# leggedrobotics/raisimLib

Measured on AMD Instinct MI355X. Metric: env-steps/sec, 4096 ANYmal-C envs flat terrain dt=0.0025, higher is better.
Workload: dtype f32

## Files before the change

### raisimlib_amd/csrc/rsb_world.hip

```cpp
#include <dlfcn.h>
#include <hip/hip_runtime.h>

#include <algorithm>
#include <cmath>
#include <cstdio>
#include <cstdlib>
#include <chrono>
#include <cstring>
#include <memory>
#include <string>
#include <vector>

#include "query_kernel.h"
#include "rsb.h"
#include "rsb_internal.h"
#include "step_launch.h"
#include "env_task.h"
#include "step_types.h"


#include "rsb_world.h"
#include "rsb_spec.h"

namespace rsbw {

struct DevKernargDefault { DevKernargDefault() { setenv("HIP_FORCE_DEV_KERNARG", "1", 0); setenv("GPU_MAX_HW_QUEUES", "8", 0); } } g_dev_kernarg_default;

int round4(int x) { return (x + 3) & ~3; }

void build_dev_model(const rsb_model_blob& b, DevModel* d) {
  std::memset(d, 0, sizeof *d);
  d->nb = b.nb; d->nq = b.nq; d->nv = b.nv; d->ncol = b.ncol; d->depth = b.depth;
  d->cw = round4(6 + b.depth - 1);
  d->fixed_base = b.fixed_base;
  std::vector<std::vector<int>> kids(b.nb);
  for (int i = 0; i < b.nb; ++i) {
    d->parent[i] = b.parent[i]; d->level[i] = b.level[i]; d->jtype[i] = b.jtype[i];
    if (i > 0) kids[b.parent[i]].push_back(i);
    float* f = d->bodyf[i];
    for (int c = 0; c < 3; ++c) {
      d->axis[i][c] = f[c] = (float)b.axis[i][c];
      d->ptree[i][c] = f[4 + c] = (float)b.ptree[i][c];
      d->com[i][c] = f[17 + c] = (float)b.com[i][c];
    }
    std::memcpy(&f[3], &b.jtype[i], sizeof(int));
    for (int c = 0; c < 9; ++c) d->rtree[i][c] = f[8 + c] = (float)b.rtree[i][c];
    for (int c = 0; c < 6; ++c) d->inertia[i][c] = f[20 + c] = (float)b.inertia[i][c];
    d->mass[i] = f[7] = (float)b.mass[i];
    d->armature[i] = f[26] = (float)b.armature[i];
    f[27] = (float)b.damping[i];
    f[28] = (float)b.effort[i];
    const bool limited = i > 0 && b.q_lower[i] < b.q_upper[i] && b.q_lower[i] > -1e29 && b.q_upper[i] < 1e29;
    f[29] = limited ? (float)b.q_lower[i] : -3e38f;
    f[30] = limited ? (float)b.q_upper[i] : 3e38f;
  }
  for (int i = 0; i < b.nb * b.depth; ++i) d->anc[i] = -1;
  for (int i = 0; i < b.nb; ++i)
    for (int j = i; j >= 0; j = b.parent[j]) d->anc[i * b.depth + b.level[j]] = j;
  int pos = 0;
  d->max_kid = 0;
  for (int i = 0; i < b.nb; ++i) {
    d->kid_start[i] = pos;
    d->kid_count[i] = (int)kids[i].size();
    for (int c : kids[i]) d->kid_list[pos++] = c;
    if (i >= 1 && d->kid_count[i] > d->max_kid) d->max_kid = d->kid_count[i];
  }
  for (int s = 0; s < b.ncol; ++s) {
    d->col_body[s] = b.col_body[s];
    for (int c = 0; c < 3; ++c) d->col_pos[s][c] = (float)b.col_pos[s][c];
    d->col_pos[s][3] = (float)b.col_radius[s];
  }
}

std::vector<int> enumerate_self_pairs(const rsb_model_blob& b, const std::vector<uint8_t>& ignore) {
  std::vector<int> out;
  for (int i = 0; i < b.ncol; ++i)
    for (int j = i + 1; j < b.ncol; ++j) {
      const int bi = b.col_body[i], bj = b.col_body[j];
      if (bi == bj || b.parent[bi] == bj || b.parent[bj] == bi) continue;
      if (b.col_rim[i] > 0.0 || b.col_rim[j] > 0.0) continue;
      if (!(b.col_radius[i] + b.col_radius[j] > 0.0)) continue;
      if (!ignore.empty() && (ignore[bi * b.nb + bj] || ignore[bj * b.nb + bi])) continue;
      out.push_back(i); out.push_back(j);
    }
  return out;
}

int up_quad_table(const rsb_model_blob& b, int* table) {
  if (b.nb > 16 || b.depth < 2 || b.nb - 1 != 4 * (b.depth - 1)) return 0;
  int first[4], n1 = 0;
  for (int i = 1; i < b.nb; ++i) {
    if (b.level[i] == 1) { if (n1 == 4) return 0; first[n1++] = i; }
    else if (b.parent[i] != i - 1) return 0;
  }
  if (n1 != 4) return 0;
  for (int g = 0; g < 4; ++g)
    for (int lv = 1; lv < b.depth; ++lv) {
      const int body = first[g] + lv - 1;
      if (body >= b.nb || b.level[body] != lv) return 0;
      if (table) table[(lv - 1) * 4 + g] = body;
    }
  return b.depth - 1;
}

int hm_slots_for(const rsb_model_blob& b) { return std::max(rsbk::kHmSlots, (int)b.ncol); }

int kcap_of(const rsb_model_blob& b, int kmax) { return (kmax <= 8 && b.depth - 1 <= 4) ? 8 : 16; }

static LdsLayout make_layout_pitch(const rsb_model_blob& b, int kcap, int n_self, int model_pitch) {
  LdsLayout L;
  L.model_pitch = model_pitch;
  const int cw = round4(6 + b.depth - 1);
  int o = 0;
  auto take = [&](int n) { int r = o; o += round4(n); return r; };
  L.t_model = take(b.nb * model_pitch);
  L.t_gain = take(2 * b.nb);
  L.t_parlv = take(b.nb);
  L.t_anc = take(b.nb * b.depth);
  L.t_dir = take(64);
  L.t_col = take(rsbk::kColSlot * b.ncol);
  L.t_kids = take(b.nb);
  L.t_kidx = take(b.nb);
  L.t_spair = take(n_self > 0 ? n_self + 1 : 0);
  L.shared_total = o;
  o = 0;
  L.q = take(b.nq < 8 ? 8 : b.nq); L.u = take(b.nv < 8 ? 8 : b.nv);
  L.pt = take(b.nq); L.dtg = take(b.nv); L.tf = take(b.nv < 8 ? 8 : b.nv);
  L.body = take(b.nb * rsbk::kBodySlot);
  const bool tri = kcap > 8;
  if (!tri) L.fact = take(b.nb * rsbk::kFactSlot);
  L.wb = take(b.nv);
  L.con = take(kcap * rsbk::kConSlot);
  L.wc = take(3 * kcap * cw);
  L.cv = take(3 * kcap);
  L.gstride = 4 * kcap + 4;
  static_assert(rsbk::g_row_pitch(8) <= 3 * (4 * 8 + 4), "the block rows of the Delassus phase must fit the region of the dense rows");
  const int gsize = tri ? (kcap * (kcap + 1) / 2) * 12 : 3 * kcap * L.gstride;
  const int upsize = b.nb * rsbk::kUpSlot + (tri ? b.nb * rsbk::kFactSlot : 0);
  L.g = take(std::max({gsize, upsize, (rsbk::kHmRec + 8) * hm_slots_for(b) + RSB_MAX_COLLISIONS + 16}));
  if (tri) L.fact = L.g + b.nb * rsbk::kUpSlot;
  L.ginv = take(12 * kcap);
  L.lam = take(3 * kcap);
  L.warm = take(6 * b.ncol);
  L.tact = take(b.nv);
  L.cen = L.wc; L.selft = 0;
  if (n_self > 0) {
    if (4 * b.ncol > 3 * kcap * cw) L.cen = take(4 * b.ncol);
    L.selft = take(4 * kcap);
  }
  L.per_env = o + rsbk::kEnvPad;
  return L;
}

static size_t lds_bytes_of(const LdsLayout& L, int lpe) { return sizeof(float) * ((size_t)L.shared_total + (size_t)(64 / lpe) * L.per_env); }

LdsLayout make_layout(const rsb_model_blob& b, int kcap, int n_self) {
  const LdsLayout tight = make_layout_pitch(b, kcap, n_self, rsbk::kModelSlot), wide = make_layout_pitch(b, kcap, n_self, rsbk::kModelPitch);
  auto wgs = [](const LdsLayout& L, int lpe) {
    const size_t bytes = lds_bytes_of(L, lpe);
    return bytes > 160 * 1024 ? 0 : (int)std::min<size_t>(4, (160 * 1024) / bytes);
  };
  for (int lpe : {16, 32, 64}) if (wgs(wide, lpe) != wgs(tight, lpe)) return tight;
  return wide;
}

size_t lds_bytes_for(const rsb_model_blob& b, int kcap, int lpe, int n_self) { return lds_bytes_of(make_layout(b, kcap, n_self), lpe); }

int default_lpe(const rsb_model_blob& b, int kmax, int n_self) {
  const int kcap = kcap_of(b, kmax);
  const int need = b.nb > 16 ? (b.nb > 32 ? 64 : 32) : 16;
  int best = 64, best_envs = 0, best_wgs = 0;
  for (int lpe = need; lpe <= 64; lpe *= 2) {
    const size_t wg = lds_bytes_for(b, kcap, lpe, n_self);
    if (wg > 160 * 1024) continue;
    if (n_self > 30 * lpe) continue;
    const int wgs = (int)std::min<size_t>(4, (160 * 1024) / wg);
    const int envs = wgs * (64 / lpe);
    if (envs > best_envs || (envs == best_envs && wgs > best_wgs)) { best_envs = envs; best_wgs = wgs; best = lpe; }
  }
  return best;
}

__global__ void warm_clear_kernel(float* warm, const uint8_t* mask, int N, int n6) {
  const int i = blockIdx.x * blockDim.x + threadIdx.x;
  if (i >= N * n6) return;
// ... 192 lines not shown

std::vector<float> build_lds_image(const rsb_world* w, const LdsLayout& L, bool rk4_contact) {
  const rsb_model_blob& b = w->blob;
  auto dm = std::make_unique<DevModel>();
  build_dev_model(b, dm.get());
  std::vector<float> img((size_t)L.shared_total, 0.f);
  auto put_i = [&](int off, int v) { std::memcpy(&img[off], &v, sizeof(int)); };
  for (int i = 0; i < b.nb; ++i) {
    for (int c = 0; c < rsbk::kModelSlot; ++c) img[L.t_model + i * L.model_pitch + c] = dm->bodyf[i][c];
    if (rk4_contact) img[L.t_model + i * L.model_pitch + 28] = 0.f;
    const bool pd = w->control_mode == RSB_PD_PLUS_FEEDFORWARD_TORQUE && !rk4_contact && i >= 1;
    img[L.t_gain + 2 * i] = pd ? w->h_kp[i + 5] : 0.f;
    img[L.t_gain + 2 * i + 1] = pd ? w->h_kd[i + 5] : 0.f;
    put_i(L.t_parlv + i, (b.parent[i] + 1) | (b.level[i] << 8));
    put_i(L.t_kids + i, dm->kid_list[i]);
    put_i(L.t_kidx + i, dm->kid_start[i] | (dm->kid_count[i] << 16));
  }
  for (int i = 0; i < b.nb * b.depth; ++i) put_i(L.t_anc + i, dm->anc[i]);
  for (int k = 0; k < 16; ++k) {
    const double lo = ((k + 15) & 15) * 0.125 * M_PI, hi = ((k + 1) & 15) * 0.125 * M_PI;
    img[L.t_dir + 4 * k] = (float)std::cos(lo); img[L.t_dir + 4 * k + 1] = (float)std::sin(lo);
    img[L.t_dir + 4 * k + 2] = (float)std::cos(hi); img[L.t_dir + 4 * k + 3] = (float)std::sin(hi);
  }
  for (int i = 0; i < b.ncol; ++i) {
    float* ct = &img[L.t_col + rsbk::kColSlot * i];
    ct[0] = (float)b.col_pos[i][0]; ct[1] = (float)b.col_pos[i][1]; ct[2] = (float)b.col_pos[i][2]; ct[3] = (float)b.col_radius[i];
    put_i(L.t_col + rsbk::kColSlot * i + 4, b.col_body[i]);
    ct[8] = (float)b.col_axis[i][0]; ct[9] = (float)b.col_axis[i][1]; ct[10] = (float)b.col_axis[i][2]; ct[11] = (float)b.col_rim[i];
    ct[5] = (float)(w->col_mu[i] >= 0 ? w->col_mu[i] : w->mu);
    ct[6] = (float)(w->col_rest[i] >= 0 ? w->col_rest[i] : w->restitution);
    ct[7] = (float)(w->col_rthr[i] >= 0 ? w->col_rthr[i] : w->res_threshold);
  }
  for (int k = 0; k < n_self_pairs(w); ++k) put_i(L.t_spair + k, (16 * w->self_pairs[2 * k]) | ((16 * w->self_pairs[2 * k + 1]) << 16));
  return img;
}

int upload_image(rsb_world* w, const LdsLayout& L, bool rk4_contact) {
  if (!w->image_dirty && rk4_contact == w->image_rk4_contact && std::memcmp(&L, &w->image_layout, sizeof L) == 0) return RSB_OK;
    std::vector<float> img = build_lds_image(w, L, rk4_contact);
    HIP_TRY(hipMemcpyAsync(w->d_image, img.data(), img.size() * sizeof(float), hipMemcpyHostToDevice, stream_of(w)));
    const int np = n_self_pairs(w);
    std::vector<float> mat((size_t)4 * np, 0.f);
    for (int k = 0; k < np; ++k) {
      mat[4 * k] = (float)(w->self_mu[k] >= 0 ? w->self_mu[k] : w->mu);
      mat[4 * k + 1] = (float)(w->self_rest[k] >= 0 ? w->self_rest[k] : w->restitution);
      mat[4 * k + 2] = (float)(w->self_rthr[k] >= 0 ? w->self_rthr[k] : w->res_threshold);
    }
    if (np > 0) {
      if ((size_t)np > w->self_mat_cap) {
        if (w->d_self_mat) HIP_TRY(hipFree(w->d_self_mat));
        w->d_self_mat = nullptr; w->self_mat_cap = 0;
        HIP_TRY(hipMalloc(&w->d_self_mat, (size_t)4 * np * sizeof(float)));
        w->self_mat_cap = (size_t)np;
      }
      HIP_TRY(hipMemcpyAsync(w->d_self_mat, mat.data(), mat.size() * sizeof(float), hipMemcpyHostToDevice, stream_of(w)));
    }
    HIP_TRY(hipStreamSynchronize(stream_of(w)));
    w->image_dirty = false;
    w->image_layout = L; w->image_rk4_contact = rk4_contact;
  return RSB_OK;
}

void fill_world_args(const rsb_world* w, const LdsLayout& L, const StepClass& c, StepArgs& a) {
  a.model = w->d_model;
  a.gc = w->d_gc; a.gv = w->d_gv; a.ptarget = w->d_pt; a.dtarget = w->d_dt; a.tauff = w->d_tff;
#ifndef RSB_X_READ_ZERO_ROWS
  if (w->dt_zero && !w->raw_dt) a.dtarget = nullptr;
  if (w->tff_zero && !w->raw_tff) a.tauff = nullptr;
#endif
  a.kp = w->d_kp; a.kd = w->d_kd;
  a.contacts = w->d_contacts; a.contact_count = w->d_count; a.flags = w->d_flags; a.iters = w->d_iters;
  a.heights = w->d_heights;
  a.hm_index = w->d_hm_index;
  a.warm = w->warm_start ? w->d_warm : nullptr;
  a.lds_image = w->d_image; a.L = L; a.lds_floats = (int)(lds_bytes_of(L, c.lpe) / sizeof(float));
  a.gc0 = w->d_gc; a.gv0 = w->d_gv; a.reset_rows = w->N;
  a.tau_out = w->want_genf ? w->d_genf : nullptr;
  a.prof = w->d_prof;
  a.dbg = w->dbg_env >= 0 ? w->d_dbg : nullptr;
  a.dbg_env = w->dbg_env;
  a.N = w->N; a.kmax = w->kmax; a.control_mode = w->control_mode;
  a.nb = w->blob.nb; a.nq = w->blob.nq; a.nv = w->blob.nv; a.ncol = w->blob.ncol; a.depth = w->blob.depth;
  a.cw = round4(6 + w->blob.depth - 1); a.max_kid = w->max_kid; a.fixed_base = w->blob.fixed_base; a.chain = (w->chain && c.lpe == 16) ? 1 : 0;
  if (a.chain && c.kmax <= 8 && up_quad_table(w->blob, nullptr) > 0 && w->blob.nb * rsbk::kUpQuadSlot <= L.ginv - L.g) a.chain = 2;
  a.dt = (float)w->dt; a.gx = (float)w->gravity[0]; a.gy = (float)w->gravity[1]; a.gz = (float)w->gravity[2];
  a.mu = (float)w->mu; a.erp = (float)w->erp;
  a.alpha_init = (float)w->alpha_init; a.alpha_min = (float)w->alpha_min; a.alpha_decay = (float)w->alpha_decay;
  a.threshold = (float)w->threshold; a.max_iter = w->max_iter; a.section_rounds = w->section_rounds;
  a.multi_depth = w->multi_depth; a.multi_light = w->multi_light; a.multi_freeze_after = w->multi_freeze_after; a.multi_stall_window = w->multi_stall_window;
  a.anderson = w->kmax > 8 ? w->anderson : 0;
  a.anderson_clip = (float)w->anderson_clip;
  a.hm_contacts = w->hm_contacts; a.hm_second_cos = (float)w->hm_second_cos; a.hm_slots = hm_slots_for(w->blob);
  a.hm_capsule = w->hm_capsule ? w->n_cap : 0; a.hm_cap = w->d_cap;
  a.integ_theta = (float)w->integ_theta;
  a.stall_window = w->stall_window; a.stall_factor = (float)w->stall_factor; a.freeze_after = w->freeze_after; a.refine = w->refine; a.settle_tol = (float)w->settle_tol; a.restitution = (float)w->restitution; a.res_threshold = (float)w->res_threshold;
  a.terrain_type = w->terrain_type; a.hm_xs = w->hm_xs; a.hm_ys = w->hm_ys; a.ground_z = (float)w->ground_z;
  if (w->terrain_type == 1) {
    double dx = w->hm_xsize / (w->hm_xs - 1), dy = w->hm_ysize / (w->hm_ys - 1);
    a.hm_x0 = (float)(w->hm_cx - 0.5 * w->hm_xsize); a.hm_y0 = (float)(w->hm_cy - 0.5 * w->hm_ysize);
    a.hm_dx = (float)dx; a.hm_dy = (float)dy; a.hm_inv_dx = (float)(1.0 / dx); a.hm_inv_dy = (float)(1.0 / dy);
    a.hm_max = w->hm_max;
  }
  a.n_self = n_self_pairs(w); a.self_mat = w->d_self_mat;
  static const bool poison = std::getenv("RSB_POISON_LDS") != nullptr;
  a.poison_lds = poison ? 1 : 0;
  static const bool prof_fine = std::getenv("RSB_PROF_FINE") != nullptr;
  a.prof_fine = prof_fine ? 1 : 0;
}

void apply_request(rsb_world* w, const StepRequest& f, StepArgs& a) {
  if (f.rk4_contact) { a.control_mode = RSB_FORCE_AND_TORQUE; a.integ_theta = 1.f; a.tauff = w->d_tff; }
  if (f.ptarget_src) { a.ptarget = f.ptarget_src; a.ptarget_store = w->d_pt; }
  if (f.act) { a.act = f.act; a.act_mean = w->d_env_mean; a.act_std = w->env_cfg.action_std; a.ptarget_store = w->d_pt; a.tau2_out = w->d_env_tau2; }
  if (f.env_task) {
    a.env_reward = f.env_reward; a.env_ob = f.env_ob;
    a.env_fwd_coeff = w->env_cfg.forward_vel_coeff; a.env_fwd_clip = w->env_cfg.forward_vel_clip;
    a.env_torque_coeff = w->env_cfg.torque_coeff; a.env_terminal_reward = w->env_cfg.terminal_reward;
    a.tau2_out = nullptr;
  }
  a.obs_out = f.obs_out; a.obs_idx = f.obs_idx; a.obs_slots = f.obs_slots;
  if (f.peer) {
    rsb_world::Peer& P = w->peer;
    const uint32_t step = ++P.step;
    const int par = (int)(step & 1u);
    const size_t bufsz = (size_t)P.ranks * w->N * P.od;
    for (int p = 0; p < P.ranks; ++p) {
      float* pb = static_cast<float*>(P.peer_base[p]);
      a.obs_peer[p] = pb + (size_t)par * bufsz;
      a.obs_flag[p] = reinterpret_cast<uint32_t*>(pb + 2 * bufsz) + (size_t)par * RSB_MAX_RANKS + P.rank;
    }
    a.obs_ctr = reinterpret_cast<uint32_t*>(static_cast<float*>(P.base) + 2 * bufsz) + 2 * RSB_MAX_RANKS;
    a.n_obs_peers = P.ranks; a.obs_row0 = P.rank * w->N; a.obs_step = step;
    a.obs_slots = P.slots; a.obs_idx = P.idx.empty() ? nullptr : P.d_idx;
  }
  a.early_term = (w->early_term && f.have_allowed) ? 1 : 0; a.allowed = f.allowed;
  if (f.do_reset) { a.do_reset = f.do_reset; a.gc0 = f.gc0; a.gv0 = f.gv0; a.reset_rows = f.rows; }
  if (f.res_steps > 0) {
    a.res_steps = f.res_steps; a.res_full = w->res_full ? 1 : 0;
    a.res_targets = f.res_targets; a.res_period = f.res_period; a.res_first = f.res_first;
    a.res_obs_stride = f.res_obs_stride; a.res_done_stride = f.res_done_stride; a.res_pass_global0 = f.res_pass_global0;
    if (f.res_stage == 1) a.res_pol.lin = f.res_lin;
    if (f.res_stage == 2) a.res_pol.mlp = f.res_mlp;
    if (f.res_stage == 0) { a.ptarget = f.res_targets + (size_t)(f.res_first % f.res_period) * ((size_t)w->N * w->blob.nq); a.ptarget_store = w->d_pt; }
  }
  a.done_out = f.redirect_done ? f.done_out : w->d_done_out;
  a.env_mask = f.mask;
}

int enqueue_step(rsb_world* w, const StepRequest& f, bool pipelined, const StepClass& c, StepArgs& a) {
  const int blocks = (w->N + 64 / c.lpe - 1) / (64 / c.lpe);
  hipStream_t ls = nullptr;
  if (pipelined) {
    int st = pipe_begin_launch(w, a, blocks, f.closed_loop, &ls);
    if (st != RSB_OK) return st;
    if (!f.closed_loop) {
      rsb_world::PipeLog e;
      e.req = f; e.nsub = a.nsub; e.req.pipeline = false;
      if (!f.redirect_done) { e.req.redirect_done = true; e.req.done_out = w->d_done_out; }
      w->pipe_log.push_back(e);
    }
    w->pipe_time_logged += a.nsub * w->dt;
  } else {
    ls = stream_of(w);
    if (w->pipe_dep) { HIP_TRY(hipStreamWaitEvent(ls, w->pipe_dep, 0)); w->pipe_dep = nullptr; }
  }
  hipEvent_t e0 = w->ev0, e1 = w->ev1;
  const bool rec = w->timing && (w->launch_index++ % w->timing_stride == 0);
// ... 1169 lines not shown
```

### raisimlib_amd/csrc/step_kernel.h

```cpp
#pragma once

#include <hip/hip_runtime.h>
#include <stdint.h>

#include <type_traits>

#include "env_task.h"
#include "rsb_types.h"
#include "step_types.h"
#include "step_spec.h"
#include "step_math.h"
#include "step_terrain.h"
#include "step_slip.h"
#include "step_slip_pk.h"
#include "stage_bodies.h"

#ifndef RSB_X_RES_RING
#define RSB_X_RES_RING 0
#endif
#if defined(RSB_I_CL) && ((RSB_I_CL) & 64)
#define RSB_RESIDENT 1
#else
#define RSB_RESIDENT 0
#endif
// ... 145 lines not shown
    if (a.pipe_xcds > 0) {
      unsigned xcc;
      asm volatile("s_getreg_b32 %0, hwreg(HW_REG_XCC_ID)" : "=s"(xcc));
      xcc &= 15u;
      unsigned t = 0;
      if (lane == 0) t = __hip_atomic_fetch_add(a.pipe_xcc_ctr + (xcc << 6), 1u, __ATOMIC_RELAXED, __HIP_MEMORY_SCOPE_AGENT) - a.pipe_xcc_base;
      t = (unsigned)__builtin_amdgcn_readfirstlane((int)t);
      const unsigned per = gridDim.x / (unsigned)a.pipe_xcds;
      if (t >= per || xcc >= (unsigned)a.pipe_xcds) {
        if (lane == 0 && atomicCAS(a.pipe_err, 0, 1 ) == 0) __hip_atomic_store(a.pipe_err_host, 1, __ATOMIC_RELAXED, __HIP_MEMORY_SCOPE_SYSTEM);
        return;
      }
      blk = (int)(xcc * per + t);
    }
  }
  int env = blk * EPW + el;
  bool env_valid = env < a.N;
  if (!env_valid) env = a.N - 1;
  if (a.env_mask && !a.env_mask[env]) env_valid = false;
  const int nb = RSB_DIM(NB, a.nb), nq = RSB_DIM(NQ, a.nq), nv = RSB_DIM(NV, a.nv), depth = RSB_DIM(DEPTH, a.depth), ncol = RSB_DIM(NCOL, a.ncol);
#ifdef RSB_SPECIALIZED
  constexpr int cw = (6 + RSB_SPEC_DEPTH - 1 + 3) & ~3;
#else
  const int cw = a.cw;
#endif
  const bool fixed_base = RSB_DIM(FIXED_BASE, a.fixed_base != 0);
  const auto& L = a.L;

  float* MODELF = lds + L.t_model;
  float* GAIN = lds + L.t_gain;
  int* PARLV = reinterpret_cast<int*>(lds + L.t_parlv);
  int* ANC = reinterpret_cast<int*>(lds + L.t_anc);
  float* DIR16 = lds + L.t_dir;
  float* COLT = lds + L.t_col;
  int* KIDS = reinterpret_cast<int*>(lds + L.t_kids);
  int* KIDX = reinterpret_cast<int*>(lds + L.t_kidx);
  float* E = lds + L.shared_total + el * L.per_env;
  float* Q = E + L.q;
  float* U = E + L.u;
  float* PT = E + L.pt;
  float* DTG = E + L.dtg;
  float* TF = E + L.tf;
  float* BODY = E + L.body;
  float* UPS = E + L.g;
  float* FACT = E + L.fact;
  float* WB = E + L.wb;
  float* CON = E + L.con;
  float* WC = E + L.wc;
  float* CV = E + L.cv;
  float* G = E + L.g;
  float* GINV = E + L.ginv;
  float* LAM = E + L.lam;
  float* TACT = E + L.tact;
  float* WARM = E + L.warm;
  const int* SPAIR = reinterpret_cast<const int*>(lds + L.t_spair);
  float* CEN = E + L.cen;
  float* SELFT = E + L.selft;
  const int n_self = RSB_DIM(N_SELF, a.n_self);
  const int nwarm = 6 * ncol;
  const int GS = L.gstride;

  if (PROF && a.poison_lds) {
    for (int i = lane; i < a.lds_floats; i += 64) lds[i] = __int_as_float(0x7fc00000);
    __syncthreads();
  }
#if RSB_RESIDENT
#if RSB_SPEC_CONSTS
  int ncs_pin = a.res_steps;
  asm volatile("" : "+s"(ncs_pin));
  const int ncs = ncs_pin;
#else
  const int ncs = a.res_steps;
#endif
  if constexpr (STG != 0) resident_stage<STG, EPW>(ka, blk, 0, ncs);
#endif
#include "step_phase_prologue.inc"
#if RSB_SEAM_CARRY
  [[maybe_unused]] float sc_q = 0.f, sc_qd = 0.f;
  [[maybe_unused]] float sc_qv[7], sc_uv[6];
#endif
#if RSB_LEAN_SEAM
#include "step_phase_seam_setup.inc"
#endif
#if RSB_RESIDENT
  for (int cs = 0; cs < ncs; ++cs) {
#endif
#if RSB_SEAM_CARRY
#if RSB_LEAN_SEAM
  if (seam_refill)
#endif
  {
#if RSB_SEAM_BASE
    float t0[8], t1[8];
    ldv<2>(Q, t0); ldv<2>(U, t1);
#endif
#if RSB_SEAM_JOINTS
    const float jq = Q[bb + 6], jqd = U[bb + 5];
    sc_q = isbody ? jq : 0.f; sc_qd = isbody ? jqd : 0.f;
#endif
#if RSB_SEAM_BASE
    RSB_UNROLL for (int i = 0; i < 7; ++i) sc_qv[i] = t0[i];
    RSB_UNROLL for (int i = 0; i < 6; ++i) sc_uv[i] = t1[i];
#endif
  }
#endif
  for (int sub = 0; sub < nsub; ++sub) {
    RSB_STAMP(0)
    RSB_ARGS(ab);
    tsq = 0.f;
#include "step_phase_tree_down.inc"
#include "step_phase_collision.inc"
#include "step_phase_tree_up.inc"
    iters_used = 0;
    float wlam[6] = {0.f, 0.f, 0.f, 0.f, 0.f, 0.f};
    if (ncw > 0) {
      RSB_ARGS(aw);
      const float erp = RSB_DIM_F32(ERP, aw.erp);
#include "step_phase_columns.inc"
#include "step_phase_delassus.inc"
#include "step_phase_solver.inc"
    } else if (has_warm) {
      for (int i = s; i < nwarm; i += LPE) WARM[i] = 0.f;
    }
    RSB_STAMP(6)

#include "step_phase_update.inc"
  }

  if (PROF && a.prof && lane == 0) { long long* P = a.prof + 16 + 16 * (long long)blk; P[8] = t_setup; P[9] = t_newt; P[10] = t_epi; P[11] = t_rule; P[12] = t_exch; P[13] = t_end; P[14] = t_start - t_entry; P[15] = t_mag; P[0] = clock64() - t_start; P[1] = t_gs; P[2] = p_iters; P[3] = p_ncw; P[4] = p_search; P[5] = p_newton; P[6] = p_solves; P[7] = t_srch; }
#if RSB_LEAN_SEAM
  if (ls_ok && cs + 1 < ncs) {
#include "step_phase_seam_lean.inc"
  } else {
    seam_refill = true;
    asm volatile("; rsb generic seam begin");
#endif
#include "step_phase_epilogue.inc"
#if RSB_LEAN_SEAM
    asm volatile("; rsb generic seam end");
  }
#endif
#if RSB_RESIDENT
  }
#endif
}

}
```

### raisimlib_amd/csrc/step_phase_delassus.inc

```
      const int npw = ncw * (ncw + 1) / 2;
      for (int p0 = 0; p0 < npw; p0 += LPE) {
        const int p = p0 + s;
        const int j = (int)((__builtin_sqrtf(8.0f * (float)p + 1.5f) - 1.0f) * 0.5f);
        const int i = p - ((j * (j + 1)) >> 1);
        if (j < nc) {
          const int bi = __float_as_int(CON[i * kConSlot + 7]), bj = __float_as_int(CON[j * kConSlot + 7]);
          const int li = PARLV[bi] >> 8, lj = PARLV[bj] >> 8;
          int ai[ML], aj[ML];
#if defined(RSB_SPECIALIZED) && RSB_SPEC_DEPTH == 4
          {
            const int4 ri = *reinterpret_cast<const int4*>(ANC + bi * 4), rj = *reinterpret_cast<const int4*>(ANC + bj * 4);
            const int vi[4] = {ri.y, ri.z, ri.w, -1}, vj[4] = {rj.y, rj.z, rj.w, -2};
            RSB_UNROLL for (int l = 0; l < ML; ++l) {
              ai[l] = (l + 1 <= li && l < 3) ? vi[l < 3 ? l : 3] : -1;
              aj[l] = (l + 1 <= lj && l < 3) ? vj[l < 3 ? l : 3] : -2;
            }
          }
#else
          RSB_UNROLL for (int l = 0; l < ML; ++l) {
            ai[l] = (l + 1 <= li) ? ANC[bi * depth + l + 1] : -1;
            aj[l] = (l + 1 <= lj) ? ANC[bj * depth + l + 1] : -2;
          }
#endif
          int lca = 0;
          bool same = true;
          RSB_UNROLL for (int l = 0; l < ML; ++l) { same = same && (ai[l] == aj[l]); lca += same ? 1 : 0; }
#if RSB_FLAT_SETUP_HEAD
          constexpr int CWC = 6 + RSB_SPEC_DEPTH - 1;
#else
          constexpr int CWC = 6 + ML;
#endif
          float wi[3][CWC], wj[3][CWC];
          const float* Wi = WC + (3 * i) * cw;
          const float* Wj = WC + (3 * j) * cw;
          RSB_UNROLL for (int rr = 0; rr < 3; ++rr) {
            RSB_UNROLL for (int q4 = 0; q4 < (CWC + 3) / 4; ++q4) {
              float t4[4], u4[4];
              ld4(Wi + rr * cw + 4 * q4, t4); ld4(Wj + rr * cw + 4 * q4, u4);
              RSB_UNROLL for (int e = 0; e < 4; ++e)
                if (4 * q4 + e < CWC) { wi[rr][4 * q4 + e] = t4[e]; wj[rr][4 * q4 + e] = u4[e]; }
            }
          }
          float acc[9];
          RSB_UNROLL for (int q2 = 0; q2 < 9; ++q2) acc[q2] = 0.f;
          RSB_UNROLL for (int e = 0; e < CWC; ++e) {
            const bool on = e < 6 || e < 6 + lca;
            float av[3], bv[3];
            RSB_UNROLL for (int rr = 0; rr < 3; ++rr) { av[rr] = on ? wi[rr][e] : 0.f; bv[rr] = on ? wj[rr][e] : 0.f; }
            RSB_UNROLL for (int rr = 0; rr < 3; ++rr)
              RSB_UNROLL for (int cc = 0; cc < 3; ++cc) acc[3 * rr + cc] += av[rr] * bv[cc];
          }
          if (i == j && CON[i * kConSlot + 15] != 0.f) { acc[0] = 1.f; acc[4] = 1.f; }
          if constexpr (TRI) {
            float* bp = G + tri_off(j, i);
            RSB_UNROLL for (int cc = 0; cc < 3; ++cc) {
              const float row[4] = {acc[cc], acc[3 + cc], acc[6 + cc], 0.f};
              st4(bp + 4 * cc, row);
            }
          } else if constexpr (GROWS) {
            const float B[3][3] = {{acc[0], acc[1], acc[2]}, {acc[3], acc[4], acc[5]}, {acc[6], acc[7], acc[8]}};
            const float Bt[3][3] = {{acc[0], acc[3], acc[6]}, {acc[1], acc[4], acc[7]}, {acc[2], acc[5], acc[8]}};
            gblk_store(G + i * GRP + kGBlock * j, B);
            if (i != j) gblk_store(G + j * GRP + kGBlock * i, Bt);
          } else {
            RSB_UNROLL for (int rr = 0; rr < 3; ++rr)
              RSB_UNROLL for (int cc = 0; cc < 3; ++cc) {
                G[(3 * i + rr) * GS + 4 * j + cc] = acc[3 * rr + cc];
                G[(3 * j + cc) * GS + 4 * i + rr] = acc[3 * rr + cc];
              }
          }
          if (i == j) {
            float gi[12];
            inv3(acc, gi);
            gi[9] = gi[10] = gi[11] = 0.f;
            stv<3>(GINV + 12 * i, gi);
          }
        }
      }
      __syncthreads();
      if constexpr (FIXED) {
        if (s < nc && __float_as_int(CON[s * kConSlot + 11]) < kSelfA) {
          float acc[9], gi[12];
          float* dg = TRI ? G + tri_off(s, s) : (GROWS ? G + s * GRP + kGBlock * s : G + 3 * s * GS + 4 * s);
          const int dgs = TRI ? 4 : GS;
          if constexpr (GROWS) {
            float D[3][3];
            gblk_load(dg, D);
            RSB_UNROLL for (int rr = 0; rr < 3; ++rr) RSB_UNROLL for (int cc = 0; cc < 3; ++cc) acc[3 * rr + cc] = D[rr][cc];
          } else {
            RSB_UNROLL for (int rr = 0; rr < 3; ++rr) {
              float g4[4];
              ld4(dg + rr * dgs, g4);
              acc[3 * rr] = g4[0]; acc[3 * rr + 1] = g4[1]; acc[3 * rr + 2] = g4[2];
            }
          }
          const float reg = kSelfReg * (acc[0] + acc[4] + acc[8]) * (1.0f / 3.0f);
          RSB_UNROLL for (int rr = 0; rr < 3; ++rr) { acc[4 * rr] += reg; dg[GROWS ? g_block_off(rr, rr) : rr * dgs + rr] = acc[4 * rr]; }
          inv3(acc, gi);
          gi[9] = gi[10] = gi[11] = 0.f;
          stv<3>(GINV + 12 * s, gi);
        }
        __syncthreads();
      }
      if (__any(nselfc > 0)) {
        for (int sa = 0; sa + 1 < ncw; ++sa) {
          const bool prim = sa + 1 < nc && (__float_as_int(CON[sa * kConSlot + 11]) & kSelfA) != 0;
          if (!__any(prim)) continue;
          const int sb = sa + 1;
          const float z4[4] = {0.f, 0.f, 0.f, 0.f};
          if constexpr (TRI) {
            if (prim && s < nc) {
              float A[3][3], B[3][3];
              const float Z[3][3] = {{0.f, 0.f, 0.f}, {0.f, 0.f, 0.f}, {0.f, 0.f, 0.f}};
              if (s != sa && s != sb) {
                tri_load(G, sa, s, A); tri_load(G, sb, s, B);
                RSB_UNROLL for (int r = 0; r < 3; ++r) RSB_UNROLL for (int c = 0; c < 3; ++c) A[r][c] += B[r][c];
                tri_store(G, sa, s, A); tri_store(G, sb, s, Z);
              } else if (s == sa) {
                float X[3][3], D[3][3];
                tri_load(G, sa, sa, A); tri_load(G, sb, sb, B); tri_load(G, sb, sa, X);
                RSB_UNROLL for (int r = 0; r < 3; ++r) RSB_UNROLL for (int c = 0; c < 3; ++c) D[r][c] = A[r][c] + B[r][c] + X[r][c] + X[c][r];
                const float ju = SELFT[4 * sa + 3] + SELFT[4 * sb + 3];
                float m4[4];
                ld4(SELFT + 4 * sa, m4);
                RSB_UNROLL for (int rr = 0; rr < 3; ++rr) { CV[3 * sa + rr] += CV[3 * sb + rr]; CV[3 * sb + rr] = 0.f; }
                if (m4[1] > 0.f && ju < -m4[2]) CV[3 * sa + 2] += m4[1] * ju;
                const float reg = (FIXED ? 2.f : 1.f) * kSelfReg * (D[0][0] + D[1][1] + D[2][2]) * (1.0f / 3.0f);
                RSB_UNROLL for (int rr = 0; rr < 3; ++rr) D[rr][rr] += reg;
                const float I3[3][3] = {{1.f, 0.f, 0.f}, {0.f, 1.f, 0.f}, {0.f, 0.f, 1.f}};
                tri_store(G, sa, sa, D); tri_store(G, sb, sa, Z); tri_store(G, sb, sb, I3);
                float acc[9], gi[12];
                RSB_UNROLL for (int r = 0; r < 3; ++r) RSB_UNROLL for (int c = 0; c < 3; ++c) acc[3 * r + c] = D[r][c];
                inv3(acc, gi);
                gi[9] = gi[10] = gi[11] = 0.f;
                stv<3>(GINV + 12 * sa, gi);
                RSB_UNROLL for (int q2 = 0; q2 < 12; ++q2) gi[q2] = 0.f;
                gi[0] = gi[4] = gi[8] = 1.f;
                stv<3>(GINV + 12 * sb, gi);
              }
            }
            __syncthreads();
            continue;
          }
          if (prim && s < nc) {
            if constexpr (GROWS) {
              gblk_add(G + sa * GRP + kGBlock * s, G + sb * GRP + kGBlock * s);
            } else {
              RSB_UNROLL for (int rr = 0; rr < 3; ++rr) {
                float ga[4], gb[4];
                ld4(G + (3 * sa + rr) * GS + 4 * s, ga); ld4(G + (3 * sb + rr) * GS + 4 * s, gb);
                RSB_UNROLL for (int e = 0; e < 4; ++e) ga[e] += gb[e];
                st4(G + (3 * sa + rr) * GS + 4 * s, ga); st4(G + (3 * sb + rr) * GS + 4 * s, z4);
              }
            }
          }
          __syncthreads();
          if constexpr (GROWS) {
            if (prim && s < nc) gblk_add(G + s * GRP + kGBlock * sa, G + s * GRP + kGBlock * sb);
          } else if (prim) {
            for (int r = s; r < 3 * nc; r += LPE) {
              float ga[4], gb[4];
// ... 38 lines not shown
```

### raisimlib_amd/csrc/step_spec.h

```cpp
#pragma once

#define RSB_SPEC_FIELDS(X)                                                                                                              \
  X(NB, a.nb) X(NQ, a.nq) X(NV, a.nv) X(DEPTH, a.depth) X(NCOL, a.ncol) X(MAX_KID, a.max_kid) X(FIXED_BASE, (a.fixed_base != 0))      \
  X(N_SELF, a.n_self) X(NSUB, a.nsub) X(KMAX, a.kmax) X(HAS_WARM, (a.warm != nullptr)) X(TERRAIN, a.terrain_type)                      \
  X(EARLY_TERM, (a.early_term != 0)) X(SECTION_ROUNDS, a.section_rounds) X(STALL_WINDOW, a.stall_window) X(FREEZE_AFTER, a.freeze_after) \
  X(REFINE, a.refine) X(MULTI_FA, a.multi_freeze_after) X(MULTI_DEPTH, a.multi_depth) X(MULTI_LIGHT, a.multi_light)                    \
  X(MULTI_SW, a.multi_stall_window) X(CHAIN, (a.chain != 0)) X(MODEL_PITCH, a.L.model_pitch) \
  X(UP_QUADS, (a.chain == 2)) \
  X(MU, rsbk::spec_bits(a.mu)) X(ERP, rsbk::spec_bits(a.erp)) X(ALPHA_INIT, rsbk::spec_bits(a.alpha_init)) X(ALPHA_MIN, rsbk::spec_bits(a.alpha_min)) \
  X(ALPHA_DECAY, rsbk::spec_bits(a.alpha_decay)) X(THRESHOLD, rsbk::spec_bits(a.threshold)) X(STALL_FACTOR, rsbk::spec_bits(a.stall_factor)) \
  X(MAX_ITER, a.max_iter)

#ifdef RSB_SPECIALIZED
#define RSB_DIM(NAME, expr) (RSB_SPEC_##NAME)
#else
#define RSB_DIM(NAME, expr) (expr)
#endif

namespace rsbk {
constexpr int spec_bits(float f) { return __builtin_bit_cast(int, f); }
constexpr float spec_f32(int bits) { return __builtin_bit_cast(float, bits); }
}
#if defined(RSB_SPECIALIZED) && !defined(RSB_X_NO_SPEC_CONSTS)
#define RSB_SPEC_CONSTS 1
// ... 12 lines not shown
#endif
#else
#define RSB_UP_QUADS 0
#endif

#if RSB_UP_QUADS && !defined(RSB_X_NO_DOWN_QUADS)
#define RSB_DOWN_QUADS 1
#else
#define RSB_DOWN_QUADS 0
#endif

#if RSB_DOWN_QUADS && !defined(RSB_X_NO_SEAM_CARRY)
#define RSB_SEAM_CARRY 1
#else
#define RSB_SEAM_CARRY 0
#endif
#if RSB_SEAM_CARRY && !defined(RSB_X_NO_SEAM_JOINTS)
#define RSB_SEAM_JOINTS 1
#else
#define RSB_SEAM_JOINTS 0
#endif
#if RSB_SEAM_CARRY && !defined(RSB_X_NO_SEAM_BASE)
#define RSB_SEAM_BASE 1
#else
#define RSB_SEAM_BASE 0
#endif
#if RSB_SEAM_CARRY && !defined(RSB_X_NO_SEAM_LOADS)
#define RSB_SEAM_LOADS 1
#else
#define RSB_SEAM_LOADS 0
#endif

#if defined(RSB_SPECIALIZED) && defined(RSB_I_CL) && (RSB_I_CL) == 64 && (RSB_I_LPE) == 16 && (RSB_I_KMAX) == 8 && RSB_SPEC_NQ > 16 && RSB_SPEC_NQ <= 32 && \
    RSB_SPEC_NQ + RSB_SPEC_NV > 32 && RSB_SPEC_NQ + RSB_SPEC_NV <= 48 && !defined(RSB_X_NO_LEAN_SEAM)
#define RSB_LEAN_SEAM 1
#else
#define RSB_LEAN_SEAM 0
#endif

#if defined(RSB_SPECIALIZED) && defined(RSB_I_LPE) && (RSB_I_LPE) == 16 && (RSB_I_KMAX) <= 8 && (RSB_I_ML) <= 4 && RSB_SPEC_DEPTH >= 2 && RSB_SPEC_DEPTH <= 4 && \
    RSB_SPEC_DEPTH <= (RSB_I_ML) && ((6 + RSB_SPEC_DEPTH - 1 + 3) & ~3) > 6 + RSB_SPEC_DEPTH - 1
#define RSB_FLAT_CLASS 1
#else
#define RSB_FLAT_CLASS 0
#endif
#if RSB_FLAT_CLASS && !defined(RSB_X_NO_FLAT_CONTACT)
#define RSB_FLAT_CONTACT 1
#else
#define RSB_FLAT_CONTACT 0
#endif
#if RSB_FLAT_CONTACT && !defined(RSB_X_NO_FLAT_COLUMNS)
#define RSB_FLAT_COLUMNS 1
#else
#define RSB_FLAT_COLUMNS 0
#endif
#if RSB_FLAT_CONTACT && !defined(RSB_X_NO_FLAT_SCATTER)
#define RSB_FLAT_SCATTER 1
#else
#define RSB_FLAT_SCATTER 0
#endif
#if RSB_FLAT_CLASS
namespace rsbk {
constexpr int kFlatCw = (6 + RSB_SPEC_DEPTH - 1 + 3) & ~3, kFlatSink = kFlatCw - 1;
static_assert(kFlatSink >= 6 + RSB_SPEC_DEPTH - 1 && kFlatSink < kFlatCw, "flat contact form: the sink must be a padding entry of the column");
}
#endif

#if RSB_FLAT_CLASS && !((RSB_I_CL) & (32 | 1)) && !defined(RSB_X_G_SQUARE) && !defined(RSB_X_NO_FLAT_SETUP)
#define RSB_FLAT_SETUP 1
#else
#define RSB_FLAT_SETUP 0
#endif
#if RSB_FLAT_SETUP && !defined(RSB_X_NO_FLAT_SETUP_HEAD)
#define RSB_FLAT_SETUP_HEAD 1
#else
#define RSB_FLAT_SETUP_HEAD 0
#endif
#if RSB_FLAT_SETUP && RSB_FLAT_SCATTER && !defined(RSB_X_NO_FLAT_SETUP_END)
#define RSB_FLAT_SETUP_END 1
#else
#define RSB_FLAT_SETUP_END 0
#endif

#if defined(RSB_SPECIALIZED) && defined(RSB_I_LPE) && (RSB_I_LPE) == 16 && (RSB_I_KMAX) <= 8 && !((RSB_I_CL) & 32)
#define RSB_PK_CLASS 1
#else
#define RSB_PK_CLASS 0
#endif
#if RSB_PK_CLASS && !defined(RSB_X_NO_PK_SOLVE)
#define RSB_PK_SOLVE 1
#else
#define RSB_PK_SOLVE 0
#endif

namespace rsbk {
#define RSB_SPEC_COUNT_ONE(NAME, expr) +1
constexpr int kSpecFields = 0 RSB_SPEC_FIELDS(RSB_SPEC_COUNT_ONE);
#undef RSB_SPEC_COUNT_ONE
}
```

Measured before the change: 389.8 million.

## Add closed-form flat Delassus block assembly for quadruped chain layout

```diff
diff --git a/raisimlib_amd/csrc/rsb_world.hip b/raisimlib_amd/csrc/rsb_world.hip
--- a/raisimlib_amd/csrc/rsb_world.hip
+++ b/raisimlib_amd/csrc/rsb_world.hip
@@ -101,6 +101,25 @@
       if (table) table[(lv - 1) * 4 + g] = body;
     }
   return b.depth - 1;
+}
+
+static bool delassus_closed_form_ok(const rsb_model_blob& b) {
+  const int nl = b.depth - 1;
+  if (nl < 1) return false;
+  std::vector<int> anc((size_t)b.nb * b.depth, -1);
+  for (int i = 0; i < b.nb; ++i)
+    for (int j = i; j >= 0; j = b.parent[j]) anc[(size_t)i * b.depth + b.level[j]] = j;
+  auto level_of = [&](int x) { return x > 0 ? (x - 1) % nl + 1 : 0; };
+  for (int i = 0; i < b.nb; ++i) {
+    if (level_of(i) != b.level[i]) return false;
+    for (int j = 0; j < b.nb; ++j) {
+      int table = 0;
+      while (table < nl && table + 1 <= b.level[i] && table + 1 <= b.level[j] && anc[(size_t)i * b.depth + table + 1] == anc[(size_t)j * b.depth + table + 1]) ++table;
+      const int form = (i > 0 && j > 0 && (i - 1) / nl == (j - 1) / nl) ? std::min(level_of(i), level_of(j)) : 0;
+      if (form != table) return false;
+    }
+  }
+  return true;
 }
 
 int hm_slots_for(const rsb_model_blob& b) { return std::max(rsbk::kHmSlots, (int)b.ncol); }
@@ -459,7 +478,7 @@
   a.N = w->N; a.kmax = w->kmax; a.control_mode = w->control_mode;
   a.nb = w->blob.nb; a.nq = w->blob.nq; a.nv = w->blob.nv; a.ncol = w->blob.ncol; a.depth = w->blob.depth;
   a.cw = round4(6 + w->blob.depth - 1); a.max_kid = w->max_kid; a.fixed_base = w->blob.fixed_base; a.chain = (w->chain && c.lpe == 16) ? 1 : 0;
-  if (a.chain && c.kmax <= 8 && up_quad_table(w->blob, nullptr) > 0 && w->blob.nb * rsbk::kUpQuadSlot <= L.ginv - L.g) a.chain = 2;
+  if (a.chain && c.kmax <= 8 && up_quad_table(w->blob, nullptr) > 0 && delassus_closed_form_ok(w->blob) && w->blob.nb * rsbk::kUpQuadSlot <= L.ginv - L.g) a.chain = 2;
   a.dt = (float)w->dt; a.gx = (float)w->gravity[0]; a.gy = (float)w->gravity[1]; a.gz = (float)w->gravity[2];
   a.mu = (float)w->mu; a.erp = (float)w->erp;
   a.alpha_init = (float)w->alpha_init; a.alpha_min = (float)w->alpha_min; a.alpha_decay = (float)w->alpha_decay;
diff --git a/raisimlib_amd/csrc/step_kernel.h b/raisimlib_amd/csrc/step_kernel.h
--- a/raisimlib_amd/csrc/step_kernel.h
+++ b/raisimlib_amd/csrc/step_kernel.h
@@ -251,6 +251,13 @@
 #if RSB_LEAN_SEAM
 #include "step_phase_seam_setup.inc"
 #endif
+#if RSB_FLAT_DELASSUS
+  int fd_j = (int)((__builtin_sqrtf(8.0f * (float)s + 1.5f) - 1.0f) * 0.5f);
+  int fd_i = s - ((fd_j * (fd_j + 1)) >> 1);
+  int fd_wi = 3 * fd_i * cw, fd_wj = 3 * fd_j * cw;
+  int fd_ob = fd_i * GRP + kGBlock * fd_j, fd_ot = fd_j * GRP + kGBlock * fd_i, fd_og = 12 * fd_i;
+  asm volatile("" : "+v"(fd_i), "+v"(fd_j), "+v"(fd_wi), "+v"(fd_wj), "+v"(fd_ob), "+v"(fd_ot), "+v"(fd_og));
+#endif
 #if RSB_RESIDENT
   for (int cs = 0; cs < ncs; ++cs) {
 #endif
diff --git a/raisimlib_amd/csrc/step_phase_delassus.inc b/raisimlib_amd/csrc/step_phase_delassus.inc
--- a/raisimlib_amd/csrc/step_phase_delassus.inc
+++ b/raisimlib_amd/csrc/step_phase_delassus.inc
@@ -1,4 +1,74 @@
+#if RSB_FLAT_CLASS
+      asm volatile("; rsb delassus begin");
+#endif
       const int npw = ncw * (ncw + 1) / 2;
+#if RSB_FLAT_DELASSUS
+      static_assert(GROWS && !TRI && !FIXED && LPE == 16 && KMAX == 8 && RSB_SPEC_DEPTH - 1 <= ML, "flat Delassus form: the row-block layout of the floating-base quadruped classes");
+      static_assert(3 * KMAX * (4 * KMAX + 4) - KMAX * GRP >= 64, "flat Delassus form: the sink lies behind the block rows, inside the region");
+      float* const fsink = G + KMAX * GRP + 16 * (s & 3);
+      int fpi = fd_i, fpj = fd_j, fwi = fd_wi, fwj = fd_wj, fob = fd_ob, fot = fd_ot, fog = fd_og;
+      for (int p0 = 0;;) {
+        const bool has = fpj < nc, diag = fpi == fpj;
+        const int i = has ? fpi : 0, j = has ? fpj : 0;
+        const float* Wi = WC + (has ? fwi : 0);
+        const float* Wj = WC + (has ? fwj : 0);
+#if RSB_FLAT_SETUP_HEAD
+        constexpr int CWC = 6 + RSB_SPEC_DEPTH - 1;
+#else
+        constexpr int CWC = 6 + ML;
+#endif
+        float wi[3][CWC], wj[3][CWC];
+        RSB_UNROLL for (int rr = 0; rr < 3; ++rr) {
+          RSB_UNROLL for (int q4 = 0; q4 < (CWC + 3) / 4; ++q4) {
+            float t4[4], u4[4];
+            ld4(Wi + rr * cw + 4 * q4, t4); ld4(Wj + rr * cw + 4 * q4, u4);
+            RSB_UNROLL for (int e = 0; e < 4; ++e)
+              if (4 * q4 + e < CWC) { wi[rr][4 * q4 + e] = t4[e]; wj[rr][4 * q4 + e] = u4[e]; }
+          }
+        }
+        const float cbi = CON[i * kConSlot + 7], clim = CON[i * kConSlot + 15], cbj = CON[j * kConSlot + 7];
+        __builtin_amdgcn_sched_barrier(0);
+        constexpr unsigned NL = RSB_SPEC_DEPTH - 1;
+        const int bi = __float_as_int(cbi), bj = __float_as_int(cbj);
+        const unsigned ui = (unsigned)(bi - 1), uj = (unsigned)(bj - 1), gi_ = ui / NL, gj_ = uj / NL;
+        const int li = bi > 0 ? (int)(ui - gi_ * NL) + 1 : 0, lj = bj > 0 ? (int)(uj - gj_ * NL) + 1 : 0;
+        const int lca = gi_ == gj_ ? min(li, lj) : 0;
+        float acc[9];
+        RSB_UNROLL for (int q2 = 0; q2 < 9; ++q2) acc[q2] = 0.f;
+        RSB_UNROLL for (int e = 0; e < CWC; ++e) {
+          const bool on = e < 6 || e < 6 + lca;
+          float av[3], bv[3];
+          RSB_UNROLL for (int rr = 0; rr < 3; ++rr) { av[rr] = on ? wi[rr][e] : 0.f; bv[rr] = on ? wj[rr][e] : 0.f; }
+          RSB_UNROLL for (int rr = 0; rr < 3; ++rr)
+            RSB_UNROLL for (int cc = 0; cc < 3; ++cc) acc[3 * rr + cc] += av[rr] * bv[cc];
+        }
+        const bool lim = diag & (clim != 0.f);
+        acc[0] = lim ? 1.f : acc[0]; acc[4] = lim ? 1.f : acc[4];
+        const float B[3][3] = {{acc[0], acc[1], acc[2]}, {acc[3], acc[4], acc[5]}, {acc[6], acc[7], acc[8]}};
+        const float Bt[3][3] = {{acc[0], acc[3], acc[6]}, {acc[1], acc[4], acc[7]}, {acc[2], acc[5], acc[8]}};
+        gblk_store(has ? G + fob : fsink, B);
+        gblk_store(has ? G + fot : fsink, Bt);
+        float gi[12];
+        {
+          const float* A = acc;
+          auto cof = [](float x, float y, float z, float w) { return fmaf(x, y, -(z * w)); };
+          const float c0 = cof(A[4], A[8], A[5], A[7]), c1 = cof(A[5], A[6], A[3], A[8]), c2 = cof(A[3], A[7], A[4], A[6]);
+          const float id = 1.0f / fmaf(A[2], c2, fmaf(A[0], c0, A[1] * c1));
+          gi[0] = c0 * id; gi[1] = cof(A[2], A[7], A[1], A[8]) * id; gi[2] = cof(A[1], A[5], A[2], A[4]) * id;
+          gi[3] = c1 * id; gi[4] = cof(A[0], A[8], A[2], A[6]) * id; gi[5] = cof(A[2], A[3], A[0], A[5]) * id;
+          gi[6] = c2 * id; gi[7] = cof(A[1], A[6], A[0], A[7]) * id; gi[8] = cof(A[0], A[4], A[1], A[3]) * id;
+        }
+        gi[9] = gi[10] = gi[11] = 0.f;
+        stv<3>((has & diag) ? GINV + fog : fsink, gi);
+        p0 += LPE;
+        if (__builtin_expect(p0 >= npw, 1)) break;
+        const int p = p0 + s;
+        fpj = (int)((__builtin_sqrtf(8.0f * (float)p + 1.5f) - 1.0f) * 0.5f);
+        fpi = p - ((fpj * (fpj + 1)) >> 1);
+        fwi = 3 * fpi * cw; fwj = 3 * fpj * cw;
+        fob = fpi * GRP + kGBlock * fpj; fot = fpj * GRP + kGBlock * fpi; fog = 12 * fpi;
+      }
+#else
       for (int p0 = 0; p0 < npw; p0 += LPE) {
         const int p = p0 + s;
         const int j = (int)((__builtin_sqrtf(8.0f * (float)p + 1.5f) - 1.0f) * 0.5f);
@@ -77,6 +147,10 @@
           }
         }
       }
+#endif
+#if RSB_FLAT_CLASS
+      asm volatile("; rsb delassus end");
+#endif
       __syncthreads();
       if constexpr (FIXED) {
         if (s < nc && __float_as_int(CON[s * kConSlot + 11]) < kSelfA) {
diff --git a/raisimlib_amd/csrc/step_spec.h b/raisimlib_amd/csrc/step_spec.h
--- a/raisimlib_amd/csrc/step_spec.h
+++ b/raisimlib_amd/csrc/step_spec.h
@@ -118,6 +118,12 @@
 #define RSB_FLAT_SETUP_END 0
 #endif
 
+#if RSB_FLAT_SETUP && (RSB_I_KMAX) == 8 && RSB_SPEC_UP_QUADS && !defined(RSB_X_NO_FLAT_DELASSUS)
+#define RSB_FLAT_DELASSUS 1
+#else
+#define RSB_FLAT_DELASSUS 0
+#endif
+
 #if defined(RSB_SPECIALIZED) && defined(RSB_I_LPE) && (RSB_I_LPE) == 16 && (RSB_I_KMAX) <= 8 && !((RSB_I_CL) & 32)
 #define RSB_PK_CLASS 1
 #else
```

Result: faster. 395.5 million (median of 6 runs) (+1.5%).
